# rail-berkeley/serl

Hardware: NVIDIA H100
Metric: drq_critic_grad_steps_per_sec (higher is better)
Workload: dtype f16

## Files before the change

serl_b200/csrc/conv3x3_res.cu:

```cuda
#include "common.cuh"
#include "conv_common.cuh"
#include "serl_b200.h"
#include "wgmma.cuh"

namespace serl {

template <int W, int CI>
struct R3Cfg {
  static constexpr int ROWS = 256 / W;
  static constexpr int BANDS = W / ROWS;
  static constexpr int PARTS = BANDS * (CI / 64);
  static constexpr int CB = CI / 64;
  static constexpr int NBOX = 3 * CB;
  static constexpr int STAGES = CB == 1 ? 3 : 2;
  static constexpr int BOX = W * (ROWS + 2) * 128;
  static constexpr int WTILES = 9 * CB;
  static constexpr int CG = CI / 4;
  static constexpr int NG = 64 / CG;
  static constexpr int WPG = CG / 16;
  static constexpr int PF = 4;
  static constexpr int OFF_A = WTILES * 8192;
  static constexpr int OFF_STG = OFF_A + STAGES * BOX;
  static constexpr int OFF_RED = OFF_STG + 8 * 1024;
  static constexpr int OFF_SLOT = OFF_RED + 2 * 4 * 2 * 4;
// ... 257 lines not shown
  }
  TcEncodeTiledFn enc = tc_get_encode();
  if (!enc) { set_last_error("serl_conv3x3_res_h16: cuTensorMapEncodeTiled unavailable"); return SERL_ERR_CUDA; }
  const CUtensorMapDataType dt = d->fmt == SERL_FMT_FP16 ? CU_TENSOR_MAP_DATA_TYPE_FLOAT16 : CU_TENSOR_MAP_DATA_TYPE_BFLOAT16;
  CUtensorMap xmap, wmap;
  {
    const cuuint64_t gdim[4] = {(cuuint64_t)CI, (cuuint64_t)W, (cuuint64_t)W, (cuuint64_t)d->N};
    const cuuint64_t gstr[3] = {(cuuint64_t)CI * 2, (cuuint64_t)W * CI * 2, (cuuint64_t)W * W * CI * 2};
    const cuuint32_t box[4] = {64u, (cuuint32_t)W, (cuuint32_t)(K::ROWS + 2), 1u};
    const cuuint32_t estr[4] = {1u, 1u, 1u, 1u};
    CUresult r = enc(&xmap, dt, 4, const_cast<void*>(d->x), gdim, gstr, box, estr, CU_TENSOR_MAP_INTERLEAVE_NONE, CU_TENSOR_MAP_SWIZZLE_128B,
                     CU_TENSOR_MAP_L2_PROMOTION_L2_256B, CU_TENSOR_MAP_FLOAT_OOB_FILL_NONE);
    if (r != CUDA_SUCCESS) { set_last_error("serl_conv3x3_res_h16: cuTensorMapEncodeTiled (input) failed (%d)", (int)r); return SERL_ERR_CUDA; }
  }
  {
    const cuuint64_t gdim[2] = {(cuuint64_t)9 * CI, (cuuint64_t)CI};
    const cuuint64_t gstr[1] = {(cuuint64_t)9 * CI * 2};
    const cuuint32_t box[2] = {64u, 64u};
    const cuuint32_t estr[2] = {1u, 1u};
    CUresult r = enc(&wmap, dt, 2, const_cast<void*>(d->w), gdim, gstr, box, estr, CU_TENSOR_MAP_INTERLEAVE_NONE, CU_TENSOR_MAP_SWIZZLE_128B,
                     CU_TENSOR_MAP_L2_PROMOTION_L2_256B, CU_TENSOR_MAP_FLOAT_OOB_FILL_NONE);
    if (r != CUDA_SUCCESS) { set_last_error("serl_conv3x3_res_h16: cuTensorMapEncodeTiled (weights) failed (%d)", (int)r); return SERL_ERR_CUDA; }
  }
  Res3Args a{};
  a.y = static_cast<uint16_t*>(d->y); a.res = static_cast<const uint16_t*>(d->res); a.gamma = d->gamma; a.beta = d->beta;
  a.res_stats = d->res_stats; a.res_gamma = d->res_gamma; a.res_beta = d->res_beta;
  a.error = d->error; a.N = d->N; a.relu = d->relu; a.eps = d->eps;
  const int rounds = ceil_div(d->N, groups);
  const int used = ceil_div(d->N, rounds);
  launch_k_cluster(kern, dim3(used * K::PARTS), dim3(CONV_THREADS), K::BANDS, (size_t)K::SMEM, st, xmap, wmap, a);
  return check_launch("conv3x3_res_kernel");
}

template <int WO, int CI>
struct S2Cfg {
  static constexpr int CO = 2 * CI;
  static constexpr int BN = WO == 4 ? 128 : 64;
  static constexpr int M = 256 * 64 / BN;
  static constexpr int HW = WO * WO;
  static constexpr int IMGS = M / HW;
  static constexpr int NSL = CO / BN;
  static constexpr int CB = CI / 64;
  static constexpr bool TALL = WO >= 8;
  static constexpr int BROWS = TALL ? WO + 1 : WO;
  static constexpr int NB = TALL ? 6 : 9;
  static constexpr int NBOX = NB * CB;
  static constexpr int BOX = IMGS * BROWS * WO * 128;
  static constexpr int TILE = BN * 128;
  static constexpr int STAGE = BOX + (TALL ? 3 : 2) * TILE;
  static constexpr int STAGES = TALL ? 3 : 4;
  static constexpr int CG = CO / 4;
  static constexpr int CGS = CG < 64 ? CG : 64;
  static constexpr int GPS = 64 / CGS;
  static constexpr int NGC = BN / CG;
  static constexpr int OFF_STG = STAGES * STAGE;
  static constexpr int OFF_PAR = OFF_STG + 8 * 1024;
  static constexpr int OFF_RED = OFF_PAR + BN * 16;
  static constexpr int OFF_ST = OFF_RED + 8 * 2 * GPS * 16;
  static constexpr int OFF_BAR = OFF_ST + IMGS * NGC * 16;
  static constexpr int SMEM = OFF_BAR + 8 * 2 * STAGES + 1024;
  static_assert(BN % CG == 0, "conv3x3s2_res_kernel: an item holds whole GroupNorm groups");
  static_assert(M % HW == 0 && (BOX % 1024) == 0 && (STAGE % 1024) == 0 && SMEM <= 232448, "conv3x3s2_res_kernel: shared memory layout");
  __device__ static constexpr int m_off(int wg, int h) { return BN == 64 ? wg * 128 + h * 64 : wg * 64; }
  __device__ static constexpr int n_off(int h) { return BN == 64 ? 0 : h * 64; }
};

struct S2Args {
  uint16_t* y; uint16_t* r; const float* gamma; const float* beta; const float* gamma_p; const float* beta_p;
  int32_t* error; int N; float eps;
};

template <class F, int WO, int CI>
__global__ void __launch_bounds__(CONV_THREADS, 1)
conv3x3s2_res_kernel(const __grid_constant__ CUtensorMap xmap, const __grid_constant__ CUtensorMap wmap,
                     const __grid_constant__ CUtensorMap pmap, const S2Args a) {
  pdl_prologue();
  using K = S2Cfg<WO, CI>;
  extern __shared__ uint8_t smem_raw[];
  uint8_t* smem = reinterpret_cast<uint8_t*>((reinterpret_cast<uintptr_t>(smem_raw) + 1023) & ~(uintptr_t)1023);
  float* par = reinterpret_cast<float*>(smem + K::OFF_PAR);
  float* red = reinterpret_cast<float*>(smem + K::OFF_RED);
  float* gst = reinterpret_cast<float*>(smem + K::OFF_ST);
  uint64_t* full = reinterpret_cast<uint64_t*>(smem + K::OFF_BAR);
  uint64_t* empty = full + K::STAGES;

  const int warp = threadIdx.x >> 5, lane = threadIdx.x & 31;
  const int n_items = ceil_div(a.N, K::IMGS) * K::NSL;

  if (threadIdx.x == 0) {
    for (int s = 0; s < K::STAGES; ++s) { tc_mbar_init(&full[s], 1); tc_mbar_init(&empty[s], 8); }
    asm volatile("fence.mbarrier_init.release.cluster;" ::: "memory");
  }
  __syncthreads();

  if (warp >= 8) {
    asm volatile("setmaxnreg.dec.sync.aligned.u32 40;" ::: "memory");
    if (warp == 8 && lane == 0) {
      asm volatile("prefetch.tensormap [%0];" ::"l"(&xmap) : "memory");
      asm volatile("prefetch.tensormap [%0];" ::"l"(&wmap) : "memory");
      asm volatile("prefetch.tensormap [%0];" ::"l"(&pmap) : "memory");
      bool ok = true;
      int it = 0;
      for (int item = blockIdx.x; item < n_items && ok; item += gridDim.x) {
        const int img = (item / K::NSL) * K::IMGS, n0 = (item % K::NSL) * K::BN;
        for (int b = 0; b < K::NBOX; ++b, ++it) {
          const int s = it % K::STAGES;
          ok = tc_mbar_wait(&empty[s], ((uint32_t)(it / K::STAGES) & 1u) ^ 1u, a.error);
          if (!ok) break;
          const int cb = b / K::NB, row = (b % K::NB) / 3, sx = b % 3;
          const int ntap = K::TALL && row == 0 ? 2 : 1;
          const bool proj = row == 0 && sx == 0;
          uint8_t* st = smem + s * K::STAGE;
          tc_mbar_expect_tx(&full[s], (uint32_t)(K::BOX + (ntap + (int)proj) * K::TILE));
          tc_tma_4d(st, &xmap, cb * 64, sx, row, img, &full[s]);
          for (int t = 0; t < ntap; ++t) {
            const int r = row + 2 * t;
            tc_tma_2d(st + K::BOX + t * K::TILE, &wmap, ((r * 3 + sx) * K::CB + cb) * 64, n0, &full[s]);
          }
          if (proj) tc_tma_2d(st + K::BOX + ntap * K::TILE, &pmap, cb * 64, n0, &full[s]);
        }
      }
    }
  } else {
    asm volatile("setmaxnreg.inc.sync.aligned.u32 232;" ::: "memory");
    const int tid = threadIdx.x, wg = tid >> 7, wl = warp & 3;
    const uint32_t s_base = smem_u32(smem);
    uint32_t a_off[2], b_off[2];
#pragma unroll
    for (int h = 0; h < 2; ++h) {
      const int m = K::m_off(wg, h);
      a_off[h] = (uint32_t)(((m / K::HW) * K::BROWS * WO + m % K::HW) * 128);
      b_off[h] = (uint32_t)(K::n_off(h) * 128);
    }
    const float count = (float)K::HW * (float)K::CG;
    bool ok = true;
    int it = 0;
    float acc[2][32], pacc[2][32];
    for (int item = blockIdx.x; item < n_items && ok; item += gridDim.x) {
      const int img0 = (item / K::NSL) * K::IMGS, n0 = (item % K::NSL) * K::BN;
      for (int cb = 0; cb < K::CB && ok; ++cb) {
#pragma unroll
        for (int bb = 0; bb < K::NB; ++bb, ++it) {
          const int s = it % K::STAGES;
          ok = tc_mbar_wait(&full[s], (uint32_t)(it / K::STAGES) & 1u, a.error);
          if (!ok) break;
          const int row = bb / 3, sx = bb % 3;
          const int ntap = K::TALL && row == 0 ? 2 : 1;
          const uint32_t as = s_base + (uint32_t)(s * K::STAGE), ws = as + (uint32_t)K::BOX;
          wg_fence();
#pragma unroll
          for (int t = 0; t < ntap; ++t)
#pragma unroll
            for (int k = 0; k < 4; ++k)
#pragma unroll
              for (int h = 0; h < 2; ++h)
                wg_mma_h16<F::kBf16>(acc[h], wg_desc(as + a_off[h] + (uint32_t)(t * WO * 128)) + 2 * k,
                                     wg_desc(ws + (uint32_t)(t * K::TILE) + b_off[h]) + 2 * k, (uint32_t)(cb | bb | t | k));
          if (row == 0 && sx == 0) {
#pragma unroll
            for (int k = 0; k < 4; ++k)
#pragma unroll
              for (int h = 0; h < 2; ++h)
                wg_mma_h16<F::kBf16>(pacc[h], wg_desc(as + a_off[h]) + 2 * k, wg_desc(ws + (uint32_t)(ntap * K::TILE) + b_off[h]) + 2 * k,
                                     (uint32_t)(cb | k));
          }
          wg_commit();
          if (cb > 0 || bb > 0) {
            wg_wait<1>();
            __syncwarp();
            if (lane == 0) tc_mbar_arrive(&empty[(it - 1) % K::STAGES]);
          }
        }
      }
      wg_wait<0>();
      ok = mma_bar_and(ok);
      if (!ok) break;
      __syncwarp();
      if (lane == 0) tc_mbar_arrive(&empty[(it - 1) % K::STAGES]);

#pragma unroll
      for (int h = 0; h < 2; ++h)
#pragma unroll
        for (int g = 0; g < K::GPS; ++g) {
          float v[4] = {0.f, 0.f, 0.f, 0.f};
#pragma unroll
          for (int j = g * K::CGS / 8; j < (g + 1) * K::CGS / 8; ++j) {
            const float* d = &acc[h][4 * j];
            const float* p = &pacc[h][4 * j];
            v[0] += (d[0] + d[1]) + (d[2] + d[3]);
            v[1] += (d[0] * d[0] + d[1] * d[1]) + (d[2] * d[2] + d[3] * d[3]);
            v[2] += (p[0] + p[1]) + (p[2] + p[3]);
            v[3] += (p[0] * p[0] + p[1] * p[1]) + (p[2] * p[2] + p[3] * p[3]);
          }
#pragma unroll
          for (int q = 0; q < 4; ++q) {
            v[q] = warp_sum(v[q]);
// ... 53 lines not shown
            for (int e = lane; e < 64; e += 32) {
              const int q = e >> 3, ch = e & 7;
              const uint4 v = *reinterpret_cast<const uint4*>(stg + q * 128 + ((ch ^ q) << 4));
              *reinterpret_cast<uint4*>(out + (pix0 + q) * K::CO + n0 + K::n_off(h) + ch * 8) = v;
            }
            __syncwarp();
          }
        }
    }
  }
}

template <class F, int WO, int CI>
static int launch_conv3x3s2_res(const serl_conv3x3s2_res_desc* d, cudaStream_t st) {
  using K = S2Cfg<WO, CI>;
  auto kern = conv3x3s2_res_kernel<F, WO, CI>;
  static int slots = 0;
  if (!slots) {
    if (cudaFuncSetAttribute(kern, cudaFuncAttributeMaxDynamicSharedMemorySize, K::SMEM) != cudaSuccess) return check_launch("cudaFuncSetAttribute(conv3x3s2_res)");
    int dev = 0, sms = 0, per_sm = 0;
    cudaGetDevice(&dev);
    cudaDeviceGetAttribute(&sms, cudaDevAttrMultiProcessorCount, dev);
    if (cudaOccupancyMaxActiveBlocksPerMultiprocessor(&per_sm, kern, CONV_THREADS, K::SMEM) != cudaSuccess) return check_launch("cudaOccupancyMaxActiveBlocksPerMultiprocessor(conv3x3s2_res)");
    if (per_sm <= 0) { set_last_error("serl_conv3x3s2_res_h16: conv3x3s2_res_kernel (%d B shared memory) cannot be resident", K::SMEM); return SERL_ERR_CUDA; }
    slots = per_sm * sms;
  }
  TcEncodeTiledFn enc = tc_get_encode();
  if (!enc) { set_last_error("serl_conv3x3s2_res_h16: cuTensorMapEncodeTiled unavailable"); return SERL_ERR_CUDA; }
  const CUtensorMapDataType dt = d->fmt == SERL_FMT_FP16 ? CU_TENSOR_MAP_DATA_TYPE_FLOAT16 : CU_TENSOR_MAP_DATA_TYPE_BFLOAT16;
  CUtensorMap xmap, wmap, pmap;
  {
    const cuuint64_t gdim[4] = {(cuuint64_t)CI, (cuuint64_t)(2 * WO), (cuuint64_t)(2 * WO), (cuuint64_t)d->N};
    const cuuint64_t gstr[3] = {(cuuint64_t)CI * 2, (cuuint64_t)2 * WO * CI * 2, (cuuint64_t)4 * WO * WO * CI * 2};
    const cuuint32_t box[4] = {64u, (cuuint32_t)(2 * WO), (cuuint32_t)(2 * K::BROWS), (cuuint32_t)K::IMGS};
    const cuuint32_t estr[4] = {1u, 2u, 2u, 1u};
    CUresult r = enc(&xmap, dt, 4, const_cast<void*>(d->x), gdim, gstr, box, estr, CU_TENSOR_MAP_INTERLEAVE_NONE, CU_TENSOR_MAP_SWIZZLE_128B,
                     CU_TENSOR_MAP_L2_PROMOTION_L2_256B, CU_TENSOR_MAP_FLOAT_OOB_FILL_NONE);
    if (r != CUDA_SUCCESS) { set_last_error("serl_conv3x3s2_res_h16: cuTensorMapEncodeTiled (input) failed (%d)", (int)r); return SERL_ERR_CUDA; }
  }
  for (int pj = 0; pj < 2; ++pj) {
    const cuuint64_t kdim = (cuuint64_t)(pj ? 1 : 9) * CI;
    const cuuint64_t gdim[2] = {kdim, (cuuint64_t)K::CO};
    const cuuint64_t gstr[1] = {kdim * 2};
    const cuuint32_t box[2] = {64u, (cuuint32_t)K::BN};
    const cuuint32_t estr[2] = {1u, 1u};
    CUresult r = enc(pj ? &pmap : &wmap, dt, 2, const_cast<void*>(pj ? d->w_proj : d->w), gdim, gstr, box, estr, CU_TENSOR_MAP_INTERLEAVE_NONE,
                     CU_TENSOR_MAP_SWIZZLE_128B, CU_TENSOR_MAP_L2_PROMOTION_L2_256B, CU_TENSOR_MAP_FLOAT_OOB_FILL_NONE);
    if (r != CUDA_SUCCESS) { set_last_error("serl_conv3x3s2_res_h16: cuTensorMapEncodeTiled (weights) failed (%d)", (int)r); return SERL_ERR_CUDA; }
  }
  S2Args a{};
  a.y = static_cast<uint16_t*>(d->y); a.r = static_cast<uint16_t*>(d->r);
  a.gamma = d->gamma; a.beta = d->beta; a.gamma_p = d->gamma_proj; a.beta_p = d->beta_proj;
  a.error = d->error; a.N = d->N; a.eps = d->eps;
  const int items = ceil_div(d->N, K::IMGS) * K::NSL;
  const int rounds = ceil_div(items, slots);
  launch_k(kern, dim3(ceil_div(items, rounds)), dim3(CONV_THREADS), (size_t)K::SMEM, st, xmap, wmap, pmap, a);
  return check_launch("conv3x3s2_res_kernel");
}

template <int W, int CI>
struct DeepCfg {
  static constexpr int BN = 128;
  static constexpr int HW = W * W;
  static constexpr int IMGS = 256 / HW;
  static constexpr int NSL = CI / BN;
  static constexpr int CB = CI / 64;
  static constexpr bool TALL = W == 8;
  static constexpr int BROWS = TALL ? W + 2 : W;
  static constexpr int NB = TALL ? 3 : 9;
  static constexpr int NTAP = TALL ? 3 : 1;
  static constexpr int NBOX = NB * CB;
  static constexpr int BOX = IMGS * BROWS * W * 128;
  static constexpr int TILE = BN * 128;
  static constexpr int STAGE = BOX + NTAP * TILE;
  static constexpr int STAGES = TALL ? 2 : 4;
  static constexpr int RES = 128 * 128 * 2;
  static constexpr int RPS = STAGE / RES;
  static constexpr int NRES = 2 / RPS;
  static constexpr int CG = CI / 4;
  static constexpr int NGC = BN / CG;
  static constexpr int OFF_STG = STAGES * STAGE;
  static constexpr int OFF_PAR = OFF_STG + 8 * 2048;
  static constexpr int OFF_RED = OFF_PAR + BN * 16;
  static constexpr int OFF_ST = OFF_RED + 8 * 2 * 2 * 8;
  static constexpr int OFF_BAR = OFF_ST + IMGS * NGC * 16;
  static constexpr int SMEM = OFF_BAR + 8 * 2 * STAGES + 1024;
  static_assert(CG >= 64 && BN % CG == 0, "conv3x3_deep_kernel: an n64 sub-tile lies in one group, an item holds whole groups");
  static_assert(RPS >= 1 && NRES < STAGES, "conv3x3_deep_kernel: the residual fits the ring");
  static_assert(HW >= 16 && (BOX % 1024) == 0 && (STAGE % 1024) == 0 && SMEM <= 232448, "conv3x3_deep_kernel: shared memory layout");
  __device__ static constexpr int m_off(int wg, int h) { return wg * 128 + h * 64; }
};

struct DeepArgs {
  uint16_t* y; float* out_f32; const uint16_t* res; const float* gamma; const float* beta;
  const float* res_stats; const float* res_gamma; const float* res_beta;
  int32_t* error; int N, relu; float eps;
};

template <class F, int W, int CI>
__global__ void __launch_bounds__(CONV_THREADS, 1)
conv3x3_deep_kernel(const __grid_constant__ CUtensorMap xmap, const __grid_constant__ CUtensorMap wmap,
                    const __grid_constant__ CUtensorMap rmap, const DeepArgs a) {
  pdl_prologue();
  using K = DeepCfg<W, CI>;
  extern __shared__ uint8_t smem_raw[];
  uint8_t* smem = reinterpret_cast<uint8_t*>((reinterpret_cast<uintptr_t>(smem_raw) + 1023) & ~(uintptr_t)1023);
  float* par = reinterpret_cast<float*>(smem + K::OFF_PAR);
  float* red = reinterpret_cast<float*>(smem + K::OFF_RED);
// ... 4 lines not shown
  const int warp = threadIdx.x >> 5, lane = threadIdx.x & 31;
  const int n_items = ceil_div(a.N, K::IMGS) * K::NSL;

  if (threadIdx.x == 0) {
    for (int s = 0; s < K::STAGES; ++s) { tc_mbar_init(&full[s], 1); tc_mbar_init(&empty[s], 8); }
    asm volatile("fence.mbarrier_init.release.cluster;" ::: "memory");
  }
  __syncthreads();

  if (warp >= 8) {
    asm volatile("setmaxnreg.dec.sync.aligned.u32 40;" ::: "memory");
    if (warp == 8 && lane == 0) {
      asm volatile("prefetch.tensormap [%0];" ::"l"(&xmap) : "memory");
      asm volatile("prefetch.tensormap [%0];" ::"l"(&wmap) : "memory");
      if (a.res) asm volatile("prefetch.tensormap [%0];" ::"l"(&rmap) : "memory");
      bool ok = true;
      int it = 0;
      for (int item = blockIdx.x; item < n_items && ok; item += gridDim.x) {
        const int img = (item / K::NSL) * K::IMGS, n0 = (item % K::NSL) * K::BN;
        for (int b = 0; b < K::NBOX + (a.res ? K::NRES : 0); ++b, ++it) {
          const int s = it % K::STAGES;
          ok = tc_mbar_wait(&empty[s], ((uint32_t)(it / K::STAGES) & 1u) ^ 1u, a.error);
          if (!ok) break;
          uint8_t* st = smem + s * K::STAGE;
          if (b >= K::NBOX) {
            tc_mbar_expect_tx(&full[s], (uint32_t)(K::RPS * K::RES));
            for (int q = 0; q < K::RPS; ++q)
              for (int c = 0; c < 2; ++c)
                tc_tma_2d(st + q * K::RES + c * (K::RES / 2), &rmap, n0 + c * 64, img * K::HW + ((b - K::NBOX) * K::RPS + q) * 128, &full[s]);
            continue;
          }
          const int cb = b / K::NB, row = (b % K::NB) / 3, sx = b % 3;
          tc_mbar_expect_tx(&full[s], (uint32_t)K::STAGE);
          tc_tma_4d(st, &xmap, cb * 64, sx - 1, K::TALL ? -1 : row - 1, img, &full[s]);
          for (int t = 0; t < K::NTAP; ++t) {
            const int r = K::TALL ? t : row;
            tc_tma_2d(st + K::BOX + t * K::TILE, &wmap, ((r * 3 + sx) * K::CB + cb) * 64, n0, &full[s]);
          }
        }
      }
    }
  } else {
    asm volatile("setmaxnreg.inc.sync.aligned.u32 232;" ::: "memory");
    const int tid = threadIdx.x, wg = tid >> 7, wl = warp & 3;
    const uint32_t s_base = smem_u32(smem);
    uint32_t a_off[2];
#pragma unroll
    for (int h = 0; h < 2; ++h) {
      const int m = K::m_off(wg, h);
      a_off[h] = (uint32_t)(((m / K::HW) * K::BROWS * W + m % K::HW) * 128);
    }
    const float count = (float)K::HW * (float)K::CG;
    bool ok = true;
    int it = 0;
    float acc[2][2][32];
    for (int item = blockIdx.x; item < n_items && ok; item += gridDim.x) {
      const int img0 = (item / K::NSL) * K::IMGS, n0 = (item % K::NSL) * K::BN;
      for (int cb = 0; cb < K::CB && ok; ++cb) {
#pragma unroll
        for (int bb = 0; bb < K::NB; ++bb, ++it) {
          const int s = it % K::STAGES;
          ok = tc_mbar_wait(&full[s], (uint32_t)(it / K::STAGES) & 1u, a.error);
          if (!ok) break;
          const uint32_t as = s_base + (uint32_t)(s * K::STAGE), ws = as + (uint32_t)K::BOX;
          wg_fence();
#pragma unroll
          for (int t = 0; t < K::NTAP; ++t)
#pragma unroll
            for (int k = 0; k < 4; ++k)
#pragma unroll
              for (int h = 0; h < 2; ++h)
#pragma unroll
                for (int c = 0; c < 2; ++c)
                  wg_mma_h16<F::kBf16>(acc[h][c], wg_desc(as + a_off[h] + (uint32_t)(t * W * 128)) + 2 * k,
                                       wg_desc(ws + (uint32_t)(t * K::TILE + c * 64 * 128)) + 2 * k, (uint32_t)(cb | bb | t | k));
          wg_commit();
          if (cb > 0 || bb > 0) {
            wg_wait<1>();
            __syncwarp();
            if (lane == 0) tc_mbar_arrive(&empty[(it - 1) % K::STAGES]);
          }
        }
      }
      wg_wait<0>();
      ok = mma_bar_and(ok);
      if (!ok) break;
      __syncwarp();
      if (lane == 0) tc_mbar_arrive(&empty[(it - 1) % K::STAGES]);

#pragma unroll
      for (int h = 0; h < 2; ++h)
#pragma unroll
        for (int c = 0; c < 2; ++c) {
          float v0 = 0.f, v1 = 0.f;
#pragma unroll
          for (int j = 0; j < 8; ++j) {
            const float* d = &acc[h][c][4 * j];
            v0 += (d[0] + d[1]) + (d[2] + d[3]);
            v1 += (d[0] * d[0] + d[1] * d[1]) + (d[2] * d[2] + d[3] * d[3]);
          }
          v0 = warp_sum(v0); v1 = warp_sum(v1);
          if (lane == 0) *reinterpret_cast<float2*>(red + ((warp * 2 + h) * 2 + c) * 2) = make_float2(v0, v1);
        }
      asm volatile("bar.sync 1, 256;" ::: "memory");
      if (tid < K::BN) {
        const int ch = n0 + tid;
        *reinterpret_cast<float4*>(par + tid * 4) = a.res_stats ? make_float4(a.gamma[ch], a.beta[ch], a.res_gamma[ch], a.res_beta[ch])
                                                                : make_float4(a.gamma[ch], a.beta[ch], 1.f, 0.f);
// ... 81 lines not shown
          }
        }
      if (a.res) {
        __syncwarp();
        if (lane == 0)
          for (int p = 0; p < K::NRES; ++p) tc_mbar_arrive(&empty[(it + p) % K::STAGES]);
        it += K::NRES;
      }
    }
  }
}

template <class F, int W, int CI>
static int launch_conv3x3_deep(const serl_conv3x3_res_desc* d, cudaStream_t st) {
  using K = DeepCfg<W, CI>;
  auto kern = conv3x3_deep_kernel<F, W, CI>;
  static int slots = 0;
  if (!slots) {
    if (cudaFuncSetAttribute(kern, cudaFuncAttributeMaxDynamicSharedMemorySize, K::SMEM) != cudaSuccess) return check_launch("cudaFuncSetAttribute(conv3x3_deep)");
    int dev = 0, sms = 0, per_sm = 0;
    cudaGetDevice(&dev);
    cudaDeviceGetAttribute(&sms, cudaDevAttrMultiProcessorCount, dev);
    if (cudaOccupancyMaxActiveBlocksPerMultiprocessor(&per_sm, kern, CONV_THREADS, K::SMEM) != cudaSuccess) return check_launch("cudaOccupancyMaxActiveBlocksPerMultiprocessor(conv3x3_deep)");
    if (per_sm <= 0) { set_last_error("serl_conv3x3_res_h16: conv3x3_deep_kernel (%d B shared memory) cannot be resident", K::SMEM); return SERL_ERR_CUDA; }
    slots = per_sm * sms;
  }
  TcEncodeTiledFn enc = tc_get_encode();
  if (!enc) { set_last_error("serl_conv3x3_res_h16: cuTensorMapEncodeTiled unavailable"); return SERL_ERR_CUDA; }
  const CUtensorMapDataType dt = d->fmt == SERL_FMT_FP16 ? CU_TENSOR_MAP_DATA_TYPE_FLOAT16 : CU_TENSOR_MAP_DATA_TYPE_BFLOAT16;
  CUtensorMap xmap, wmap, rmap;
  {
    const cuuint64_t gdim[4] = {(cuuint64_t)CI, (cuuint64_t)W, (cuuint64_t)W, (cuuint64_t)d->N};
    const cuuint64_t gstr[3] = {(cuuint64_t)CI * 2, (cuuint64_t)W * CI * 2, (cuuint64_t)W * W * CI * 2};
    const cuuint32_t box[4] = {64u, (cuuint32_t)W, (cuuint32_t)K::BROWS, (cuuint32_t)K::IMGS};
    const cuuint32_t estr[4] = {1u, 1u, 1u, 1u};
    CUresult r = enc(&xmap, dt, 4, const_cast<void*>(d->x), gdim, gstr, box, estr, CU_TENSOR_MAP_INTERLEAVE_NONE, CU_TENSOR_MAP_SWIZZLE_128B,
                     CU_TENSOR_MAP_L2_PROMOTION_L2_256B, CU_TENSOR_MAP_FLOAT_OOB_FILL_NONE);
    if (r != CUDA_SUCCESS) { set_last_error("serl_conv3x3_res_h16: cuTensorMapEncodeTiled (input) failed (%d)", (int)r); return SERL_ERR_CUDA; }
  }
  {
    const cuuint64_t gdim[2] = {(cuuint64_t)9 * CI, (cuuint64_t)CI};
    const cuuint64_t gstr[1] = {(cuuint64_t)9 * CI * 2};
    const cuuint32_t box[2] = {64u, (cuuint32_t)K::BN};
    const cuuint32_t estr[2] = {1u, 1u};
    CUresult r = enc(&wmap, dt, 2, const_cast<void*>(d->w), gdim, gstr, box, estr, CU_TENSOR_MAP_INTERLEAVE_NONE, CU_TENSOR_MAP_SWIZZLE_128B,
                     CU_TENSOR_MAP_L2_PROMOTION_L2_256B, CU_TENSOR_MAP_FLOAT_OOB_FILL_NONE);
    if (r != CUDA_SUCCESS) { set_last_error("serl_conv3x3_res_h16: cuTensorMapEncodeTiled (weights) failed (%d)", (int)r); return SERL_ERR_CUDA; }
  }
  rmap = wmap;
  if (d->res) {
    const cuuint64_t gdim[2] = {(cuuint64_t)CI, (cuuint64_t)d->N * W * W};
    const cuuint64_t gstr[1] = {(cuuint64_t)CI * 2};
    const cuuint32_t box[2] = {64u, 128u};
    const cuuint32_t estr[2] = {1u, 1u};
    CUresult r = enc(&rmap, dt, 2, const_cast<void*>(d->res), gdim, gstr, box, estr, CU_TENSOR_MAP_INTERLEAVE_NONE, CU_TENSOR_MAP_SWIZZLE_128B,
                     CU_TENSOR_MAP_L2_PROMOTION_L2_256B, CU_TENSOR_MAP_FLOAT_OOB_FILL_NONE);
    if (r != CUDA_SUCCESS) { set_last_error("serl_conv3x3_res_h16: cuTensorMapEncodeTiled (residual) failed (%d)", (int)r); return SERL_ERR_CUDA; }
  }
  DeepArgs a{};
  a.out_f32 = d->out_f32; a.y = d->out_f32 ? nullptr : static_cast<uint16_t*>(d->y);
  a.res = static_cast<const uint16_t*>(d->res); a.gamma = d->gamma; a.beta = d->beta;
  a.res_stats = d->res_stats; a.res_gamma = d->res_gamma; a.res_beta = d->res_beta;
  a.error = d->error; a.N = d->N; a.relu = d->relu; a.eps = d->eps;
  const int items = ceil_div(d->N, K::IMGS) * K::NSL;
  const int rounds = ceil_div(items, slots);
  launch_k(kern, dim3(ceil_div(items, rounds)), dim3(CONV_THREADS), (size_t)K::SMEM, st, xmap, wmap, rmap, a);
  return check_launch("conv3x3_deep_kernel");
}

}

using namespace serl;

extern "C" int serl_conv3x3s2_res_h16(const serl_conv3x3s2_res_desc* d, void* stream) {
  if (!d || !d->x || !d->w || !d->w_proj || !d->y || !d->r || !d->gamma || !d->beta || !d->gamma_proj || !d->beta_proj || !d->error || d->N < 1) {
    set_last_error("serl_conv3x3s2_res_h16: invalid descriptor"); return SERL_ERR_INVALID;
  }
  if (d->Co != 2 * d->Ci) { set_last_error("serl_conv3x3s2_res_h16: Co == 2 Ci only (ResNet-10 stage heads)"); return SERL_ERR_UNSUPPORTED; }
  if (!((d->Wo == 16 && d->Co == 128) || (d->Wo == 8 && d->Co == 256) || (d->Wo == 4 && d->Co == 512))) {
    set_last_error("serl_conv3x3s2_res_h16: unsupported shape (Wo=%d, Ci=%d, Co=%d)", d->Wo, d->Ci, d->Co); return SERL_ERR_UNSUPPORTED;
  }
  const bool h = d->fmt == SERL_FMT_FP16;
  const cudaStream_t st = static_cast<cudaStream_t>(stream);
  if (d->Wo == 16) return h ? launch_conv3x3s2_res<Fp16, 16, 64>(d, st) : launch_conv3x3s2_res<Bf16, 16, 64>(d, st);
  if (d->Wo == 8) return h ? launch_conv3x3s2_res<Fp16, 8, 128>(d, st) : launch_conv3x3s2_res<Bf16, 8, 128>(d, st);
  return h ? launch_conv3x3s2_res<Fp16, 4, 256>(d, st) : launch_conv3x3s2_res<Bf16, 4, 256>(d, st);
}

extern "C" int serl_conv3x3_res_h16(const serl_conv3x3_res_desc* d, void* stream) {
  if (!d || !d->x || !d->w || !d->gamma || !d->beta || !d->error || (!d->y && !d->out_f32) || d->N < 1) {
    set_last_error("serl_conv3x3_res_h16: invalid descriptor"); return SERL_ERR_INVALID;
  }
  if ((d->res_stats != nullptr) != (d->res_gamma != nullptr) || (d->res_stats != nullptr) != (d->res_beta != nullptr) || (d->res_stats && !d->res)) {
    set_last_error("serl_conv3x3_res_h16: res_stats / res_gamma / res_beta go together (and need res)"); return SERL_ERR_INVALID;
  }
  if (d->H != d->W || d->Co != d->Ci) { set_last_error("serl_conv3x3_res_h16: square maps with Ci == Co only"); return SERL_ERR_UNSUPPORTED; }
  if (!((d->W == 32 && d->Ci == 64) || (d->W == 16 && d->Ci == 128) || (d->W == 8 && d->Ci == 256) || (d->W == 4 && d->Ci == 512))) {
    set_last_error("serl_conv3x3_res_h16: unsupported shape (H=W=%d, Ci=%d, Co=%d): ResNet-10 block shapes at 128x128 input only", d->W, d->Ci, d->Co);
    return SERL_ERR_UNSUPPORTED;
  }
  if (d->out_f32 && d->W >= 16) {
    set_last_error("serl_conv3x3_res_h16: out_f32 at 8x8 and 4x4 only"); return SERL_ERR_UNSUPPORTED;
  }
  if (d->W == 32) {
    return d->fmt == SERL_FMT_FP16 ? launch_conv3x3_res<Fp16, 32, 64>(d, static_cast<cudaStream_t>(stream))
                                   : launch_conv3x3_res<Bf16, 32, 64>(d, static_cast<cudaStream_t>(stream));
  }
  if (d->W == 16) {
    return d->fmt == SERL_FMT_FP16 ? launch_conv3x3_res<Fp16, 16, 128>(d, static_cast<cudaStream_t>(stream))
                                   : launch_conv3x3_res<Bf16, 16, 128>(d, static_cast<cudaStream_t>(stream));
  }
  if (d->W == 8) {
    return d->fmt == SERL_FMT_FP16 ? launch_conv3x3_deep<Fp16, 8, 256>(d, static_cast<cudaStream_t>(stream))
                                   : launch_conv3x3_deep<Bf16, 8, 256>(d, static_cast<cudaStream_t>(stream));
  }
  return d->fmt == SERL_FMT_FP16 ? launch_conv3x3_deep<Fp16, 4, 512>(d, static_cast<cudaStream_t>(stream))
                                 : launch_conv3x3_deep<Bf16, 4, 512>(d, static_cast<cudaStream_t>(stream));
}
```

Measured before the change: 476.5.

## Add ping-pong consumer conv kernel for stride-2 heads and 8x8 residual blocks

Introduces a new conv3x3_pp_kernel in which the two consumer warpgroups alternate work items (ping-pong) and each issues n256 wgmma over 256 output pixels. Named barriers order their MMA phases so one group's GroupNorm epilogue overlaps the other's tensor-core work. It is used for the Wo=16/8 stride-2 heads (projection branch split into a separate phase) and for the 8x8 residual conv. The remaining legacy kernels drop their tall-box multi-tap paths and return to one tap per stage. The cost is more complex scheduling, a 128-float accumulator per thread and register pressure.

```diff
diff --git a/serl_b200/csrc/conv3x3_res.cu b/serl_b200/csrc/conv3x3_res.cu
--- a/serl_b200/csrc/conv3x3_res.cu
+++ b/serl_b200/csrc/conv3x3_res.cu
@@ -313,25 +313,369 @@
   return check_launch("conv3x3_res_kernel");
 }
 
+template <int S, int WO, int CI>
+struct PPCfg {
+  static constexpr int CO = S * CI;
+  static constexpr int HW = WO * WO;
+  static constexpr int IMGS = 256 / HW;
+  static constexpr int NSL = CO / 64;
+  static constexpr int CB = CI / 64;
+  static constexpr int NB = S == 2 ? 6 : 3;
+  static constexpr int NPH = S == 2 ? 2 : 1;
+  static constexpr int BROWS = WO + (S == 2 ? 1 : 2);
+  static constexpr int SHIFT = IMGS * WO * 128;
+  static constexpr int BOX = BROWS * SHIFT;
+  static constexpr int STAGE = BOX + (S == 2 ? 2 : 3) * 8192;
+  static constexpr int STAGES = S == 2 ? 4 : 3;
+  static constexpr int CG = CO / 4;
+  static constexpr int WPG = CG / 16;
+  static constexpr int PF = 4;
+  static constexpr int OFF_STG = STAGES * STAGE;
+  static constexpr int OFF_RED = OFF_STG + 8 * 1024;
+  static constexpr int OFF_BAR = OFF_RED + 2 * 2 * 4 * IMGS * 2 * 4;
+  static constexpr int SMEM = OFF_BAR + 8 * 2 * STAGES + 1024;
+  static_assert(IMGS * HW == 256 && WPG <= 4 && (SHIFT % 1024) == 0 && (STAGE % 1024) == 0 && SMEM <= 232448,
+                "conv3x3_pp_kernel: shared memory layout");
+  static __host__ __device__ constexpr int nbox(int ph) { return ph ? CB : NB * CB; }
+};
+
+struct PPArgs {
+  uint16_t* y; uint16_t* r; float* out_f32; const uint16_t* res;
+  const float* gamma; const float* beta; const float* gamma_p; const float* beta_p;
+  const float* res_stats; const float* res_gamma; const float* res_beta;
+  int32_t* error; int N, relu; float eps;
+};
+
+template <class F, int S, int WO, int CI>
+__global__ void __launch_bounds__(CONV_THREADS, 1)
+conv3x3_pp_kernel(const __grid_constant__ CUtensorMap xmap, const __grid_constant__ CUtensorMap wmap,
+                  const __grid_constant__ CUtensorMap pmap, const PPArgs a) {
+  pdl_prologue();
+  using K = PPCfg<S, WO, CI>;
+  extern __shared__ uint8_t smem_raw[];
+  uint8_t* smem = reinterpret_cast<uint8_t*>((reinterpret_cast<uintptr_t>(smem_raw) + 1023) & ~(uintptr_t)1023);
+  float* red = reinterpret_cast<float*>(smem + K::OFF_RED);
+  uint64_t* full = reinterpret_cast<uint64_t*>(smem + K::OFF_BAR);
+  uint64_t* empty = full + K::STAGES;
+
+  const int warp = threadIdx.x >> 5, lane = threadIdx.x & 31;
+  const int n_items = ceil_div(a.N, K::IMGS) * K::NSL;
+  auto item_of = [&](int P) {
+    const int q = blockIdx.x + ((P & 1) + 2 * ((P >> 1) / K::NPH)) * gridDim.x;
+    return P >= 0 && q < n_items ? q : -1;
+  };
+  auto past_end = [&](int P) { return blockIdx.x + 2 * ((P >> 1) / K::NPH) * gridDim.x >= n_items; };
+
+  if (threadIdx.x == 0) {
+    for (int s = 0; s < K::STAGES; ++s) { tc_mbar_init(&full[s], 1); tc_mbar_init(&empty[s], 4); }
+    asm volatile("fence.mbarrier_init.release.cluster;" ::: "memory");
+  }
+  __syncthreads();
+
+  if (warp >= 8) {
+    asm volatile("setmaxnreg.dec.sync.aligned.u32 40;" ::: "memory");
+    if (warp == 8 && lane == 0) {
+      asm volatile("prefetch.tensormap [%0];" ::"l"(&xmap) : "memory");
+      asm volatile("prefetch.tensormap [%0];" ::"l"(&wmap) : "memory");
+      if (S == 2) asm volatile("prefetch.tensormap [%0];" ::"l"(&pmap) : "memory");
+      bool ok = true;
+      int it = 0;
+      for (int P = 0; ok && !past_end(P); ++P) {
+        const int q = item_of(P);
+        if (q < 0) continue;
+        const int ph = (P >> 1) % K::NPH;
+        const int img0 = (q / K::NSL) * K::IMGS, n0 = (q % K::NSL) * 64;
+        for (int b = 0; b < K::nbox(ph); ++b, ++it) {
+          const int s = it % K::STAGES;
+          ok = tc_mbar_wait(&empty[s], ((uint32_t)(it / K::STAGES) & 1u) ^ 1u, a.error);
+          if (!ok) break;
+          const int cb = ph ? b : b / K::NB, sx = ph ? 0 : b % 3, row0 = S == 2 && !ph ? (b % K::NB) / 3 : 0;
+          const int ntap = ph ? 1 : S == 1 ? 3 : row0 == 0 ? 2 : 1;
+          uint8_t* st = smem + s * K::STAGE;
+          tc_mbar_expect_tx(&full[s], (uint32_t)(K::BOX + ntap * 8192));
+          tc_tma_4d(st, &xmap, cb * 64, S == 2 ? sx : sx - 1, img0, S == 2 ? row0 : -1, &full[s]);
+          for (int t = 0; t < ntap; ++t) {
+            if (ph) tc_tma_2d(st + K::BOX, &pmap, cb * 64, n0, &full[s]);
+            else tc_tma_2d(st + K::BOX + t * 8192, &wmap, (((S == 2 ? row0 + 2 * t : t) * 3 + sx) * K::CB + cb) * 64, n0, &full[s]);
+          }
+        }
+      }
+    }
+  } else {
+    asm volatile("setmaxnreg.inc.sync.aligned.u32 232;" ::: "memory");
+    const int g = warp >> 2, wl = warp & 3;
+    const uint32_t s_base = smem_u32(smem);
+    const float count = (float)K::HW * (float)K::CG;
+    const int grp = wl / K::WPG;
+    const int cl = 16 * wl + (lane >> 2);
+    uint8_t* stg = smem + K::OFF_STG + warp * 1024;
+    const uint32_t mrow = smem_u32(stg) + (uint32_t)(((lane >> 4) * 8 + (lane & 7)) * 32 + ((((lane >> 3) ^ (lane >> 2)) & 1) << 4));
+    const int gpx = lane >> 1, gh = lane & 1;
+    const uint32_t grow = (uint32_t)(gpx * 32 + ((gh ^ (gpx >> 2)) & 1) * 16);
+    const int pbase = K::IMGS == 1 ? gpx : gpx & 7;
+    constexpr int RSTEP = K::IMGS == 1 ? 32 : 8, ESTEP = K::IMGS == 1 ? 16 : 0;
+    auto im_of = [&](int e) { return K::IMGS == 1 ? 0 : 2 * e + (gpx >> 3); };
+    bool ok = true;
+    int it = 0;
+    float acc[128];
+    for (int P = 0; !past_end(P); ++P) {
+      const int q = item_of(P);
+      if (q < 0) continue;
+      const int k = P >> 1, ph = k % K::NPH;
+      if ((P & 1) != g) { it += K::nbox(ph); continue; }
+      const int img0 = (q / K::NSL) * K::IMGS, n0 = (q % K::NSL) * 64;
+      if (item_of(P - 1) >= 0) named_bar_sync(2 + g, 256);
+      if (ph == 0) {
+        for (int cb = 0; cb < K::CB && ok; ++cb) {
+#pragma unroll
+          for (int bb = 0; bb < K::NB; ++bb, ++it) {
+            const int s = it % K::STAGES;
+            ok = tc_mbar_wait(&full[s], (uint32_t)(it / K::STAGES) & 1u, a.error);
+            if (!ok) break;
+            const int ntap = S == 1 ? 3 : bb < 3 ? 2 : 1;
+            const uint32_t bs = s_base + (uint32_t)(s * K::STAGE), ws = bs + (uint32_t)K::BOX;
+            wg_fence();
+#pragma unroll
+            for (int t = 0; t < ntap; ++t)
+#pragma unroll
+              for (int kk = 0; kk < 4; ++kk)
+                wg_mma_h16_n256<F::kBf16>(acc, wg_desc(ws + (uint32_t)(t * 8192)) + 2 * kk, wg_desc(bs + (uint32_t)(t * K::SHIFT)) + 2 * kk,
+                                          (uint32_t)(cb | bb | t | kk));
+            wg_commit();
+            if (cb > 0 || bb > 0) {
+              wg_wait<1>();
+              __syncwarp();
+              if (lane == 0) tc_mbar_arrive(&empty[(it - 1) % K::STAGES]);
+            }
+          }
+        }
+      } else {
+        for (int cb = 0; cb < K::CB && ok; ++cb, ++it) {
+          const int s = it % K::STAGES;
+          ok = tc_mbar_wait(&full[s], (uint32_t)(it / K::STAGES) & 1u, a.error);
+          if (!ok) break;
+          const uint32_t bs = s_base + (uint32_t)(s * K::STAGE), ws = bs + (uint32_t)K::BOX;
+          wg_fence();
+#pragma unroll
+          for (int kk = 0; kk < 4; ++kk)
+            wg_mma_h16_n256<F::kBf16>(acc, wg_desc(ws) + 2 * kk, wg_desc(bs) + 2 * kk, (uint32_t)(cb | kk));
+          wg_commit();
+          if (cb > 0) {
+            wg_wait<1>();
+            __syncwarp();
+            if (lane == 0) tc_mbar_arrive(&empty[(it - 1) % K::STAGES]);
+          }
+        }
+      }
+      if (item_of(P + 1) >= 0) named_bar_arrive(3 - g, 256);
+
+      const uint16_t* rsrc = a.res + ((size_t)img0 * K::HW + pbase) * CI + n0 + 16 * wl + 8 * gh;
+      uint4 rbuf[K::PF][2];
+      if (S == 1 && a.res && ok) {
+#pragma unroll
+        for (int p = 0; p < K::PF; ++p)
+#pragma unroll
+          for (int e = 0; e < 2; ++e)
+            rbuf[p][e] = img0 + im_of(e) < a.N ? __ldg(reinterpret_cast<const uint4*>(rsrc + (size_t)(im_of(e) * K::HW + p * RSTEP + e * ESTEP) * CI))
+                                               : make_uint4(0u, 0u, 0u, 0u);
+      }
+      wg_wait<0>();
+      __syncwarp();
+      if (ok && lane == 0) tc_mbar_arrive(&empty[(it - 1) % K::STAGES]);
+
+      float sm[K::IMGS], ss[K::IMGS];
+#pragma unroll
+      for (int im = 0; im < K::IMGS; ++im) { sm[im] = 0.f; ss[im] = 0.f; }
+#pragma unroll
+      for (int j = 0; j < 32; ++j) {
+        const float* d = &acc[4 * j];
+        sm[j % K::IMGS] += (d[0] + d[1]) + (d[2] + d[3]);
+        ss[j % K::IMGS] += (d[0] * d[0] + d[1] * d[1]) + (d[2] * d[2] + d[3] * d[3]);
+      }
+      float* rw = red + (((k & 1) * 2 + g) * 4) * K::IMGS * 2;
+#pragma unroll
+      for (int im = 0; im < K::IMGS; ++im) {
+        sm[im] = warp_sum(sm[im]); ss[im] = warp_sum(ss[im]);
+        if (lane == 0) *reinterpret_cast<float2*>(rw + (wl * K::IMGS + im) * 2) = make_float2(sm[im], ss[im]);
+      }
+      named_bar_sync(4 + g, 128);
+      if (!ok) continue;
+      float mean[K::IMGS], rstd[K::IMGS];
+#pragma unroll
+      for (int im = 0; im < K::IMGS; ++im) {
+        float s0 = 0.f, s1 = 0.f;
+#pragma unroll
+        for (int w = 0; w < K::WPG; ++w) {
+          const float2 v = *reinterpret_cast<const float2*>(rw + ((grp * K::WPG + w) * K::IMGS + im) * 2);
+          s0 += v.x; s1 += v.y;
+        }
+        mean[im] = s0 / count;
+        rstd[im] = rsqrtf(fmaxf(s1 / count - mean[im] * mean[im], 0.f) + a.eps);
+      }
+
+      const float* gam = ph ? a.gamma_p : a.gamma;
+      const float* bet = ph ? a.beta_p : a.beta;
+      const bool relu = S == 2 ? ph == 0 : a.relu != 0;
+      const bool rnorm = S == 1 && a.res_stats;
+      float ga[K::IMGS][2], gb[K::IMGS][2], ra[K::IMGS][2], rb[K::IMGS][2];
+#pragma unroll
+      for (int im = 0; im < K::IMGS; ++im) {
+        float rmean = 0.f, rrstd = 1.f;
+        if (rnorm && img0 + im < a.N) {
+          const float* rs = a.res_stats + ((size_t)(img0 + im) * 4 + n0 / K::CG) * 2;
+          rmean = rs[0] / count;
+          rrstd = rsqrtf(fmaxf(rs[1] / count - rmean * rmean, 0.f) + a.eps);
+        }
+#pragma unroll
+        for (int h = 0; h < 2; ++h) {
+          const int c = n0 + cl + 8 * h;
+          ga[im][h] = rstd[im] * gam[c];
+          gb[im][h] = bet[c] - mean[im] * ga[im][h];
+          ra[im][h] = rnorm ? rrstd * a.res_gamma[c] : 1.f;
+          rb[im][h] = rnorm ? a.res_beta[c] - rmean * ra[im][h] : 0.f;
+        }
+      }
+
+      uint16_t* out = S == 2 && ph ? a.r : a.y;
+      const size_t obase = ((size_t)img0 * K::HW + pbase) * K::CO + n0 + 16 * wl + 8 * gh;
+#pragma unroll
+      for (int rd = 0; rd < 8; ++rd) {
+        uint32_t rv[2][4];
+        if (S == 1 && a.res) {
+#pragma unroll
+          for (int e = 0; e < 2; ++e) *reinterpret_cast<uint4*>(stg + grow + e * 512) = rbuf[rd % K::PF][e];
+          __syncwarp();
+          ldsm_x4_trans(mrow, rv[0]);
+          ldsm_x4_trans(mrow + 512, rv[1]);
+          if (rd + K::PF < 8) {
+#pragma unroll
+            for (int e = 0; e < 2; ++e)
+              if (img0 + im_of(e) < a.N)
+                rbuf[rd % K::PF][e] = __ldg(reinterpret_cast<const uint4*>(rsrc + (size_t)(im_of(e) * K::HW + (rd + K::PF) * RSTEP + e * ESTEP) * CI));
+          }
+        }
+        uint32_t o[2][4];
+#pragma unroll
+        for (int x = 0; x < 2; ++x)
+#pragma unroll
+          for (int jj = 0; jj < 2; ++jj) {
+            const int j = 4 * rd + 2 * x + jj, im = j % K::IMGS;
+#pragma unroll
+            for (int h = 0; h < 2; ++h) {
+              const float* d = &acc[4 * j + 2 * h];
+              float o0 = fmaf(d[0], ga[im][h], gb[im][h]), o1 = fmaf(d[1], ga[im][h], gb[im][h]);
+              if (S == 1 && a.res) {
+                const float2 r = F::unpack(rv[x][2 * jj + h]);
+                o0 += fmaf(r.x, ra[im][h], rb[im][h]);
+                o1 += fmaf(r.y, ra[im][h], rb[im][h]);
+              }
+              if (relu) { o0 = fmaxf(o0, 0.f); o1 = fmaxf(o1, 0.f); }
+              if (S == 1 && a.out_f32 && img0 + im < a.N) {
+                float* of = a.out_f32 + ((size_t)(img0 + im) * K::HW + 8 * (j / K::IMGS) + 2 * (lane & 3)) * CI + n0 + cl + 8 * h;
+                of[0] = o0;
+                of[CI] = o1;
+              }
+              o[x][2 * jj + h] = F::pack(o0, o1);
+            }
+          }
+        __syncwarp();
+        if (S == 2 || !a.out_f32) {
+          stsm_x4_trans(mrow, o[0]);
+          stsm_x4_trans(mrow + 512, o[1]);
+          __syncwarp();
+#pragma unroll
+          for (int e = 0; e < 2; ++e)
+            if (img0 + im_of(e) < a.N)
+              *reinterpret_cast<uint4*>(out + obase + (size_t)(im_of(e) * K::HW + rd * RSTEP + e * ESTEP) * K::CO) =
+                  *reinterpret_cast<const uint4*>(stg + grow + e * 512);
+          __syncwarp();
+        }
+      }
+    }
+  }
+}
+
+template <class F, int S, int WO, int CI>
+static int launch_conv3x3_pp(const char* name, const void* x, const void* w, const void* w_proj, int fmt, const PPArgs& a, cudaStream_t st) {
+  using K = PPCfg<S, WO, CI>;
+  auto kern = conv3x3_pp_kernel<F, S, WO, CI>;
+  static int slots = 0;
+  if (!slots) {
+    if (cudaFuncSetAttribute(kern, cudaFuncAttributeMaxDynamicSharedMemorySize, K::SMEM) != cudaSuccess) return check_launch("cudaFuncSetAttribute(conv3x3_pp)");
+    int dev = 0, sms = 0, per_sm = 0;
+    cudaGetDevice(&dev);
+    cudaDeviceGetAttribute(&sms, cudaDevAttrMultiProcessorCount, dev);
+    if (cudaOccupancyMaxActiveBlocksPerMultiprocessor(&per_sm, kern, CONV_THREADS, K::SMEM) != cudaSuccess) return check_launch("cudaOccupancyMaxActiveBlocksPerMultiprocessor(conv3x3_pp)");
+    if (per_sm <= 0) { set_last_error("%s: conv3x3_pp_kernel (%d B shared memory) cannot be resident", name, K::SMEM); return SERL_ERR_CUDA; }
+    slots = per_sm * sms;
+  }
+  TcEncodeTiledFn enc = tc_get_encode();
+  if (!enc) { set_last_error("%s: cuTensorMapEncodeTiled unavailable", name); return SERL_ERR_CUDA; }
+  const CUtensorMapDataType dt = fmt == SERL_FMT_FP16 ? CU_TENSOR_MAP_DATA_TYPE_FLOAT16 : CU_TENSOR_MAP_DATA_TYPE_BFLOAT16;
+  CUtensorMap xmap, wmap, pmap;
+  {
+    constexpr int WI = S * WO;
+    const cuuint64_t gdim[4] = {(cuuint64_t)CI, (cuuint64_t)WI, (cuuint64_t)a.N, (cuuint64_t)WI};
+    const cuuint64_t gstr[3] = {(cuuint64_t)CI * 2, (cuuint64_t)WI * WI * CI * 2, (cuuint64_t)WI * CI * 2};
+    const cuuint32_t box[4] = {64u, (cuuint32_t)(S * WO), (cuuint32_t)K::IMGS, (cuuint32_t)(S * K::BROWS)};
+    const cuuint32_t estr[4] = {1u, (cuuint32_t)S, 1u, (cuuint32_t)S};
+    CUresult r = enc(&xmap, dt, 4, const_cast<void*>(x), gdim, gstr, box, estr, CU_TENSOR_MAP_INTERLEAVE_NONE, CU_TENSOR_MAP_SWIZZLE_128B,
+                     CU_TENSOR_MAP_L2_PROMOTION_L2_256B, CU_TENSOR_MAP_FLOAT_OOB_FILL_NONE);
+    if (r != CUDA_SUCCESS) { set_last_error("%s: cuTensorMapEncodeTiled (input) failed (%d)", name, (int)r); return SERL_ERR_CUDA; }
+  }
+  for (int pj = 0; pj < S; ++pj) {
+    const cuuint64_t kdim = (cuuint64_t)(pj ? 1 : 9) * CI;
+    const cuuint64_t gdim[2] = {kdim, (cuuint64_t)K::CO};
+    const cuuint64_t gstr[1] = {kdim * 2};
+    const cuuint32_t box[2] = {64u, 64u};
+    const cuuint32_t estr[2] = {1u, 1u};
+    CUresult r = enc(pj ? &pmap : &wmap, dt, 2, const_cast<void*>(pj ? w_proj : w), gdim, gstr, box, estr, CU_TENSOR_MAP_INTERLEAVE_NONE,
+                     CU_TENSOR_MAP_SWIZZLE_128B, CU_TENSOR_MAP_L2_PROMOTION_L2_256B, CU_TENSOR_MAP_FLOAT_OOB_FILL_NONE);
+    if (r != CUDA_SUCCESS) { set_last_error("%s: cuTensorMapEncodeTiled (weights) failed (%d)", name, (int)r); return SERL_ERR_CUDA; }
+  }
+  if (S == 1) pmap = wmap;
+  const int items = ceil_div(a.N, K::IMGS) * K::NSL;
+  const int rounds = ceil_div(items, slots);
+  launch_k(kern, dim3(ceil_div(items, rounds)), dim3(CONV_THREADS), (size_t)K::SMEM, st, xmap, wmap, pmap, a);
+  return check_launch("conv3x3_pp_kernel");
+}
+
+template <class F, int WO, int CI>
+static int launch_conv3x3s2_pp(const serl_conv3x3s2_res_desc* d, cudaStream_t st) {
+  PPArgs a{};
+  a.y = static_cast<uint16_t*>(d->y); a.r = static_cast<uint16_t*>(d->r);
+  a.gamma = d->gamma; a.beta = d->beta; a.gamma_p = d->gamma_proj; a.beta_p = d->beta_proj;
+  a.error = d->error; a.N = d->N; a.relu = 1; a.eps = d->eps;
+  return launch_conv3x3_pp<F, 2, WO, CI>("serl_conv3x3s2_res_h16", d->x, d->w, d->w_proj, d->fmt, a, st);
+}
+
+template <class F>
+static int launch_conv3x3_res8_pp(const serl_conv3x3_res_desc* d, cudaStream_t st) {
+  PPArgs a{};
+  a.out_f32 = d->out_f32; a.y = d->out_f32 ? nullptr : static_cast<uint16_t*>(d->y);
+  a.res = static_cast<const uint16_t*>(d->res); a.gamma = d->gamma; a.beta = d->beta;
+  a.res_stats = d->res_stats; a.res_gamma = d->res_gamma; a.res_beta = d->res_beta;
+  a.error = d->error; a.N = d->N; a.relu = d->relu; a.eps = d->eps;
+  return launch_conv3x3_pp<F, 1, 8, 256>("serl_conv3x3_res_h16", d->x, d->w, nullptr, d->fmt, a, st);
+}
+
 template <int WO, int CI>
 struct S2Cfg {
   static constexpr int CO = 2 * CI;
-  static constexpr int BN = WO == 4 ? 128 : 64;
-  static constexpr int M = 256 * 64 / BN;
+  static constexpr int BN = 128;
+  static constexpr int M = 128;
   static constexpr int HW = WO * WO;
   static constexpr int IMGS = M / HW;
   static constexpr int NSL = CO / BN;
   static constexpr int CB = CI / 64;
-  static constexpr bool TALL = WO >= 8;
-  static constexpr int BROWS = TALL ? WO + 1 : WO;
-  static constexpr int NB = TALL ? 6 : 9;
+  static constexpr int NB = 9;
   static constexpr int NBOX = NB * CB;
-  static constexpr int BOX = IMGS * BROWS * WO * 128;
+  static constexpr int BOX = IMGS * HW * 128;
   static constexpr int TILE = BN * 128;
-  static constexpr int STAGE = BOX + (TALL ? 3 : 2) * TILE;
-  static constexpr int STAGES = TALL ? 3 : 4;
+  static constexpr int STAGE = BOX + 2 * TILE;
+  static constexpr int STAGES = 4;
   static constexpr int CG = CO / 4;
-  static constexpr int CGS = CG < 64 ? CG : 64;
+  static constexpr int CGS = 64;
   static constexpr int GPS = 64 / CGS;
   static constexpr int NGC = BN / CG;
   static constexpr int OFF_STG = STAGES * STAGE;
@@ -340,10 +684,10 @@
   static constexpr int OFF_ST = OFF_RED + 8 * 2 * GPS * 16;
   static constexpr int OFF_BAR = OFF_ST + IMGS * NGC * 16;
   static constexpr int SMEM = OFF_BAR + 8 * 2 * STAGES + 1024;
-  static_assert(BN % CG == 0, "conv3x3s2_res_kernel: an item holds whole GroupNorm groups");
+  static_assert(WO == 4 && BN % CG == 0, "conv3x3s2_res_kernel: the WO 4 head, an item holds whole GroupNorm groups");
   static_assert(M % HW == 0 && (BOX % 1024) == 0 && (STAGE % 1024) == 0 && SMEM <= 232448, "conv3x3s2_res_kernel: shared memory layout");
-  __device__ static constexpr int m_off(int wg, int h) { return BN == 64 ? wg * 128 + h * 64 : wg * 64; }
-  __device__ static constexpr int n_off(int h) { return BN == 64 ? 0 : h * 64; }
+  __device__ static constexpr int m_off(int wg, int) { return wg * 64; }
+  __device__ static constexpr int n_off(int h) { return h * 64; }
 };
 
 struct S2Args {
@@ -389,16 +733,12 @@
           ok = tc_mbar_wait(&empty[s], ((uint32_t)(it / K::STAGES) & 1u) ^ 1u, a.error);
           if (!ok) break;
           const int cb = b / K::NB, row = (b % K::NB) / 3, sx = b % 3;
-          const int ntap = K::TALL && row == 0 ? 2 : 1;
           const bool proj = row == 0 && sx == 0;
           uint8_t* st = smem + s * K::STAGE;
-          tc_mbar_expect_tx(&full[s], (uint32_t)(K::BOX + (ntap + (int)proj) * K::TILE));
+          tc_mbar_expect_tx(&full[s], (uint32_t)(K::BOX + (1 + (int)proj) * K::TILE));
           tc_tma_4d(st, &xmap, cb * 64, sx, row, img, &full[s]);
-          for (int t = 0; t < ntap; ++t) {
-            const int r = row + 2 * t;
-            tc_tma_2d(st + K::BOX + t * K::TILE, &wmap, ((r * 3 + sx) * K::CB + cb) * 64, n0, &full[s]);
-          }
-          if (proj) tc_tma_2d(st + K::BOX + ntap * K::TILE, &pmap, cb * 64, n0, &full[s]);
+          tc_tma_2d(st + K::BOX, &wmap, ((row * 3 + sx) * K::CB + cb) * 64, n0, &full[s]);
+          if (proj) tc_tma_2d(st + K::BOX + K::TILE, &pmap, cb * 64, n0, &full[s]);
         }
       }
     }
@@ -410,7 +750,7 @@
 #pragma unroll
     for (int h = 0; h < 2; ++h) {
       const int m = K::m_off(wg, h);
-      a_off[h] = (uint32_t)(((m / K::HW) * K::BROWS * WO + m % K::HW) * 128);
+      a_off[h] = (uint32_t)(m * 128);
       b_off[h] = (uint32_t)(K::n_off(h) * 128);
     }
     const float count = (float)K::HW * (float)K::CG;
@@ -425,24 +765,19 @@
           const int s = it % K::STAGES;
           ok = tc_mbar_wait(&full[s], (uint32_t)(it / K::STAGES) & 1u, a.error);
           if (!ok) break;
-          const int row = bb / 3, sx = bb % 3;
-          const int ntap = K::TALL && row == 0 ? 2 : 1;
           const uint32_t as = s_base + (uint32_t)(s * K::STAGE), ws = as + (uint32_t)K::BOX;
           wg_fence();
 #pragma unroll
-          for (int t = 0; t < ntap; ++t)
+          for (int k = 0; k < 4; ++k)
+#pragma unroll
+            for (int h = 0; h < 2; ++h)
+              wg_mma_h16<F::kBf16>(acc[h], wg_desc(as + a_off[h]) + 2 * k, wg_desc(ws + b_off[h]) + 2 * k, (uint32_t)(cb | bb | k));
+          if (bb == 0) {
 #pragma unroll
             for (int k = 0; k < 4; ++k)
 #pragma unroll
               for (int h = 0; h < 2; ++h)
-                wg_mma_h16<F::kBf16>(acc[h], wg_desc(as + a_off[h] + (uint32_t)(t * WO * 128)) + 2 * k,
-                                     wg_desc(ws + (uint32_t)(t * K::TILE) + b_off[h]) + 2 * k, (uint32_t)(cb | bb | t | k));
-          if (row == 0 && sx == 0) {
-#pragma unroll
-            for (int k = 0; k < 4; ++k)
-#pragma unroll
-              for (int h = 0; h < 2; ++h)
-                wg_mma_h16<F::kBf16>(pacc[h], wg_desc(as + a_off[h]) + 2 * k, wg_desc(ws + (uint32_t)(ntap * K::TILE) + b_off[h]) + 2 * k,
+                wg_mma_h16<F::kBf16>(pacc[h], wg_desc(as + a_off[h]) + 2 * k, wg_desc(ws + (uint32_t)K::TILE + b_off[h]) + 2 * k,
                                      (uint32_t)(cb | k));
           }
           wg_commit();
@@ -562,7 +897,7 @@
   {
     const cuuint64_t gdim[4] = {(cuuint64_t)CI, (cuuint64_t)(2 * WO), (cuuint64_t)(2 * WO), (cuuint64_t)d->N};
     const cuuint64_t gstr[3] = {(cuuint64_t)CI * 2, (cuuint64_t)2 * WO * CI * 2, (cuuint64_t)4 * WO * WO * CI * 2};
-    const cuuint32_t box[4] = {64u, (cuuint32_t)(2 * WO), (cuuint32_t)(2 * K::BROWS), (cuuint32_t)K::IMGS};
+    const cuuint32_t box[4] = {64u, (cuuint32_t)(2 * WO), (cuuint32_t)(2 * WO), (cuuint32_t)K::IMGS};
     const cuuint32_t estr[4] = {1u, 2u, 2u, 1u};
     CUresult r = enc(&xmap, dt, 4, const_cast<void*>(d->x), gdim, gstr, box, estr, CU_TENSOR_MAP_INTERLEAVE_NONE, CU_TENSOR_MAP_SWIZZLE_128B,
                      CU_TENSOR_MAP_L2_PROMOTION_L2_256B, CU_TENSOR_MAP_FLOAT_OOB_FILL_NONE);
@@ -595,15 +930,12 @@
   static constexpr int IMGS = 256 / HW;
   static constexpr int NSL = CI / BN;
   static constexpr int CB = CI / 64;
-  static constexpr bool TALL = W == 8;
-  static constexpr int BROWS = TALL ? W + 2 : W;
-  static constexpr int NB = TALL ? 3 : 9;
-  static constexpr int NTAP = TALL ? 3 : 1;
+  static constexpr int NB = 9;
   static constexpr int NBOX = NB * CB;
-  static constexpr int BOX = IMGS * BROWS * W * 128;
+  static constexpr int BOX = IMGS * HW * 128;
   static constexpr int TILE = BN * 128;
-  static constexpr int STAGE = BOX + NTAP * TILE;
-  static constexpr int STAGES = TALL ? 2 : 4;
+  static constexpr int STAGE = BOX + TILE;
+  static constexpr int STAGES = 4;
   static constexpr int RES = 128 * 128 * 2;
   static constexpr int RPS = STAGE / RES;
   static constexpr int NRES = 2 / RPS;
@@ -674,11 +1006,8 @@
           }
           const int cb = b / K::NB, row = (b % K::NB) / 3, sx = b % 3;
           tc_mbar_expect_tx(&full[s], (uint32_t)K::STAGE);
-          tc_tma_4d(st, &xmap, cb * 64, sx - 1, K::TALL ? -1 : row - 1, img, &full[s]);
-          for (int t = 0; t < K::NTAP; ++t) {
-            const int r = K::TALL ? t : row;
-            tc_tma_2d(st + K::BOX + t * K::TILE, &wmap, ((r * 3 + sx) * K::CB + cb) * 64, n0, &full[s]);
-          }
+          tc_tma_4d(st, &xmap, cb * 64, sx - 1, row - 1, img, &full[s]);
+          tc_tma_2d(st + K::BOX, &wmap, ((row * 3 + sx) * K::CB + cb) * 64, n0, &full[s]);
         }
       }
     }
@@ -688,10 +1017,7 @@
     const uint32_t s_base = smem_u32(smem);
     uint32_t a_off[2];
 #pragma unroll
-    for (int h = 0; h < 2; ++h) {
-      const int m = K::m_off(wg, h);
-      a_off[h] = (uint32_t)(((m / K::HW) * K::BROWS * W + m % K::HW) * 128);
-    }
+    for (int h = 0; h < 2; ++h) a_off[h] = (uint32_t)(K::m_off(wg, h) * 128);
     const float count = (float)K::HW * (float)K::CG;
     bool ok = true;
     int it = 0;
@@ -707,15 +1033,13 @@
           const uint32_t as = s_base + (uint32_t)(s * K::STAGE), ws = as + (uint32_t)K::BOX;
           wg_fence();
 #pragma unroll
-          for (int t = 0; t < K::NTAP; ++t)
-#pragma unroll
-            for (int k = 0; k < 4; ++k)
-#pragma unroll
-              for (int h = 0; h < 2; ++h)
-#pragma unroll
-                for (int c = 0; c < 2; ++c)
-                  wg_mma_h16<F::kBf16>(acc[h][c], wg_desc(as + a_off[h] + (uint32_t)(t * W * 128)) + 2 * k,
-                                       wg_desc(ws + (uint32_t)(t * K::TILE + c * 64 * 128)) + 2 * k, (uint32_t)(cb | bb | t | k));
+          for (int k = 0; k < 4; ++k)
+#pragma unroll
+            for (int h = 0; h < 2; ++h)
+#pragma unroll
+              for (int c = 0; c < 2; ++c)
+                wg_mma_h16<F::kBf16>(acc[h][c], wg_desc(as + a_off[h]) + 2 * k, wg_desc(ws + (uint32_t)(c * 64 * 128)) + 2 * k,
+                                     (uint32_t)(cb | bb | k));
           wg_commit();
           if (cb > 0 || bb > 0) {
             wg_wait<1>();
@@ -863,7 +1187,7 @@
   {
     const cuuint64_t gdim[4] = {(cuuint64_t)CI, (cuuint64_t)W, (cuuint64_t)W, (cuuint64_t)d->N};
     const cuuint64_t gstr[3] = {(cuuint64_t)CI * 2, (cuuint64_t)W * CI * 2, (cuuint64_t)W * W * CI * 2};
-    const cuuint32_t box[4] = {64u, (cuuint32_t)W, (cuuint32_t)K::BROWS, (cuuint32_t)K::IMGS};
+    const cuuint32_t box[4] = {64u, (cuuint32_t)W, (cuuint32_t)W, (cuuint32_t)K::IMGS};
     const cuuint32_t estr[4] = {1u, 1u, 1u, 1u};
     CUresult r = enc(&xmap, dt, 4, const_cast<void*>(d->x), gdim, gstr, box, estr, CU_TENSOR_MAP_INTERLEAVE_NONE, CU_TENSOR_MAP_SWIZZLE_128B,
                      CU_TENSOR_MAP_L2_PROMOTION_L2_256B, CU_TENSOR_MAP_FLOAT_OOB_FILL_NONE);
@@ -913,8 +1237,8 @@
   }
   const bool h = d->fmt == SERL_FMT_FP16;
   const cudaStream_t st = static_cast<cudaStream_t>(stream);
-  if (d->Wo == 16) return h ? launch_conv3x3s2_res<Fp16, 16, 64>(d, st) : launch_conv3x3s2_res<Bf16, 16, 64>(d, st);
-  if (d->Wo == 8) return h ? launch_conv3x3s2_res<Fp16, 8, 128>(d, st) : launch_conv3x3s2_res<Bf16, 8, 128>(d, st);
+  if (d->Wo == 16) return h ? launch_conv3x3s2_pp<Fp16, 16, 64>(d, st) : launch_conv3x3s2_pp<Bf16, 16, 64>(d, st);
+  if (d->Wo == 8) return h ? launch_conv3x3s2_pp<Fp16, 8, 128>(d, st) : launch_conv3x3s2_pp<Bf16, 8, 128>(d, st);
   return h ? launch_conv3x3s2_res<Fp16, 4, 256>(d, st) : launch_conv3x3s2_res<Bf16, 4, 256>(d, st);
 }
 
@@ -942,8 +1266,8 @@
                                    : launch_conv3x3_res<Bf16, 16, 128>(d, static_cast<cudaStream_t>(stream));
   }
   if (d->W == 8) {
-    return d->fmt == SERL_FMT_FP16 ? launch_conv3x3_deep<Fp16, 8, 256>(d, static_cast<cudaStream_t>(stream))
-                                   : launch_conv3x3_deep<Bf16, 8, 256>(d, static_cast<cudaStream_t>(stream));
+    return d->fmt == SERL_FMT_FP16 ? launch_conv3x3_res8_pp<Fp16>(d, static_cast<cudaStream_t>(stream))
+                                   : launch_conv3x3_res8_pp<Bf16>(d, static_cast<cudaStream_t>(stream));
   }
   return d->fmt == SERL_FMT_FP16 ? launch_conv3x3_deep<Fp16, 4, 512>(d, static_cast<cudaStream_t>(stream))
                                  : launch_conv3x3_deep<Bf16, 4, 512>(d, static_cast<cudaStream_t>(stream));
```

Result: faster. 525.2 (median of 6 runs) (+10.2%).
